# abeauvisage/uasl_motion_estimation

Measured on AMD Instinct MI355X. Metric: frames/sec + BA iter/sec, 2000 feats x 20-keyframe window, 1/2/4/8 MI355X, higher is better.
Workload: dtype u8+f32 (MI), f64 (BA); 1 GPU; config 3: 1280x720 stereo, 2000 feats, 20-keyframe window, 11x11 MI patches; frame=KLT + MI scale LM (LM, MAX_NB_ITER 10, tolerances off) + 10 BA LM iterations, parallelism=1 independent streams (one per GPU)

## Files before the change

### uasl_motion_estimation_amd/csrc/ba.hip

```cpp
#include <algorithm>
#include <cmath>
#include <cstdio>
#include <cstring>
#include <mutex>
#include <numeric>
#include <vector>
#include <hip/hip_ext.h>
#include "me_internal.hpp"
#include "ba_kernels.hpp"
#include "roster.hpp"
#include "solve_diag.hpp"
#include "me_device.hpp"

using me_dev::wave_sync;

using namespace ba;

namespace {

constexpr double kDblMin = 2.2250738585072014e-308;
constexpr double kDblEps = 2.220446049250313e-16;

template <int Ctrl>
__device__ __forceinline__ double dpp_f64(double x);
// ... 231 lines not shown
  __shared__ double lds[BLK / 64];
  const State* st = b.st;
  if (st->done || !st->need_lin) return;
  const int o = blockIdx.x * BLK + threadIdx.x;
  double cost = 0;
  if (o < g.no) {
    const int cur = st->cur;
    const int ci = b.cam_idx[o], pi = b.pt_idx[o];
    double r[4], Jc[24], Jp[12];
    obs_residual<OD>(g, b, o, b.cams[cur] + 6 * ci, b.pts[cur] + 3 * pi, r, Jc, Jp);
    const double s = r[0] * r[0] + r[1] * r[1] + r[2] * r[2] + r[3] * r[3];
    double rho0, sc;
    huber(s, &rho0, &sc);
    cost = 0.5 * rho0;
    for (int k = 0; k < 4; ++k) r[k] *= sc;
    for (int k = 0; k < 24; ++k) Jc[k] *= sc;
    for (int k = 0; k < 12; ++k) Jp[k] *= sc;
    const long slot = b.pos[o];
    double* X = b.obsx + slot * kObsxStride;
    X[0] = Jp[0] * Jp[0] + Jp[3] * Jp[3] + Jp[6] * Jp[6] + Jp[9] * Jp[9];
    X[1] = Jp[0] * Jp[1] + Jp[3] * Jp[4] + Jp[6] * Jp[7] + Jp[9] * Jp[10];
    X[2] = Jp[0] * Jp[2] + Jp[3] * Jp[5] + Jp[6] * Jp[8] + Jp[9] * Jp[11];
    X[3] = Jp[1] * Jp[1] + Jp[4] * Jp[4] + Jp[7] * Jp[7] + Jp[10] * Jp[10];
    X[4] = Jp[1] * Jp[2] + Jp[4] * Jp[5] + Jp[7] * Jp[8] + Jp[10] * Jp[11];
    X[5] = Jp[2] * Jp[2] + Jp[5] * Jp[5] + Jp[8] * Jp[8] + Jp[11] * Jp[11];
    for (int a = 0; a < 3; ++a) X[6 + a] = Jp[a] * r[0] + Jp[3 + a] * r[1] + Jp[6 + a] * r[2] + Jp[9 + a] * r[3];
    if (ci - g.nf >= 0) {
      double* W = b.Wo + 18 * slot;
      for (int a = 0; a < 6; ++a)
        for (int c = 0; c < 3; ++c)
          W[a * 3 + c] = Jc[a] * Jp[c] + Jc[6 + a] * Jp[3 + c] + Jc[12 + a] * Jp[6 + c] + Jc[18 + a] * Jp[9 + c];
    }
  }
  double v[1] = {cost};
  double out[1];
  block_sum<1>(v, out, lds);
  if (threadIdx.x == 0) b.part[R_COST * g.pstride + blockIdx.x] = out[0];
}

__device__ __forceinline__ bool last_arrival_wt(unsigned* cnt, unsigned expected) {
  __shared__ int slast;
  __syncthreads();
  if (threadIdx.x == 0) {
    asm volatile("s_waitcnt vmcnt(0)" ::: "memory");
    const unsigned k = __hip_atomic_fetch_add(cnt, 1u, ME_HO_RMW, __HIP_MEMORY_SCOPE_AGENT);
    slast = k == expected - 1;
    if (slast) __hip_atomic_store(cnt, 0u, __ATOMIC_RELAXED, __HIP_MEMORY_SCOPE_AGENT);
  }
  __syncthreads();
  return slast != 0;
}

__device__ void cam_reduce_body(const Geo& g, const Bufs& b, int sharded, const double* cpart, double* colnorm,
                                double* gc_raw, double* Uraw, int ci) {
  __shared__ double tot[27];
  __shared__ double csl[6];
  const State* st = b.st;
  const int u = threadIdx.x;
  if (u < 27) {
    double sum = 0.0;
    for (int k = 0; k < g.ck; ++k) sum += a_ld<true>(&cpart[27 * ((long)ci * g.ck + k) + u]);
    tot[u] = sum;
    if (u < 21) Uraw[21 * (long)ci + u] = sum;
    else gc_raw[6 * ci + u - 21] = sum;
  }
  __syncthreads();
  if (u < 6) {
    const int d = u * 6 - u * (u - 1) / 2;
    colnorm[6 * ci + u] = tot[d];
    if (!sharded) {
      double* cs = b.csc + 6 * ci;
      if (!st->scaled) cs[u] = g.jacobi ? 1.0 / (1.0 + sqrt(tot[d])) : 1.0;
      csl[u] = cs[u];
    }
  }
  if (sharded) return;
  __syncthreads();
  if (u < 21) {
    int a = 0, r = u;
    while (r >= 6 - a) {
      r -= 6 - a;
      ++a;
    }
    const int c = a + r;
    const double x = tot[u] * csl[a] * csl[c];
    double* U = b.U + 36 * (long)ci;
    U[a * 6 + c] = x;
    U[c * 6 + a] = x;
  } else if (u < 27) {
    b.gcs[6 * ci + u - 21] = tot[u] * csl[u - 21];
  }
}

#ifdef ME_CAM_TS
__device__ unsigned long long g_cam_ts[8];
#define CAM_T(i)                                                                           \
  do {                                                                                     \
    if (ci == 0 && k == 0 && threadIdx.x == 0) {                                           \
      const long long t_ = (long long)__builtin_amdgcn_s_memtime();                        \
      if ((i) > 0) atomicAdd(&g_cam_ts[(i)], (unsigned long long)(t_ - cam_prev_));        \
      else atomicAdd(&g_cam_ts[0], 1ull);                                                  \
      cam_prev_ = t_;                                                                      \
    }                                                                                      \
  } while (0)
#else
#define CAM_T(i) \
  do {           \
  } while (0)
#endif
template <int OD>
__device__ __forceinline__ void cam_assemble_body(const Geo& g, const Bufs& b, double* cpart, int sharded,
                                                  double* colnorm, double* gc_raw, double* Uraw, int ci, int k) {
  __shared__ double rows[kBlock / 16 * 27];
  const State* st = b.st;
  if (st->done || !st->need_lin) return;
#ifdef ME_CAM_TS
  long long cam_prev_ = 0;
#endif
  CAM_T(0);
  const int beg = b.c_off[ci], end = b.c_off[ci + 1];
  double v[27];
  for (int i = 0; i < 27; ++i) v[i] = 0;
  const int cur = st->cur;
  for (int q = beg + k * kBlock + threadIdx.x; q < end; q += g.ck * kBlock) {
    const int o = b.c_obs[q];
    const int cam = b.cam_idx[o], pi = b.pt_idx[o];
    double r[4], Jc[24], Jp[12];
    obs_residual<OD>(g, b, o, b.cams[cur] + 6 * cam, b.pts[cur] + 3 * pi, r, Jc, Jp);
    const double s2 = r[0] * r[0] + r[1] * r[1] + r[2] * r[2] + r[3] * r[3];
    double rho0, sc;
    huber(s2, &rho0, &sc);
    for (int kk = 0; kk < 4; ++kk) r[kk] *= sc;
    for (int kk = 0; kk < 24; ++kk) Jc[kk] *= sc;
    int u = 0;
    for (int a = 0; a < 6; ++a)
      for (int c = a; c < 6; ++c, ++u)
        v[u] += Jc[a] * Jc[c] + Jc[6 + a] * Jc[6 + c] + Jc[12 + a] * Jc[12 + c] + Jc[18 + a] * Jc[18 + c];
    for (int a = 0; a < 6; ++a) v[21 + a] += Jc[a] * r[0] + Jc[6 + a] * r[1] + Jc[12 + a] * r[2] + Jc[18 + a] * r[3];
  }
  CAM_T(1);
#pragma unroll
  for (int u = 0; u < 27; ++u) {
    double x = v[u];
    x += dpp_f64<kDppQuadSwap1>(x);
    x += dpp_f64<kDppQuadSwap2>(x);
    x += dpp_f64<kDppRowHalfMirror>(x);
    x += dpp_f64<kDppRowMirror>(x);
    v[u] = x;
  }
  if ((threadIdx.x & 15) == 0)
#pragma unroll
    for (int u = 0; u < 27; ++u) rows[(threadIdx.x >> 4) * 27 + u] = v[u];
  __syncthreads();
  CAM_T(2);
  if (threadIdx.x < 27) {
    double sum = 0.0;
#pragma unroll
    for (int r = 0; r < kBlock / 16; ++r) sum += rows[r * 27 + threadIdx.x];
    a_st<true>(&cpart[27 * ((long)ci * g.ck + k) + threadIdx.x], sum);
  }
  const bool last = last_arrival_wt(b.cnt + ci, g.ck);
  CAM_T(3);
  if (!last) return;
  cam_reduce_body(g, b, sharded, cpart, colnorm, gc_raw, Uraw, ci);
  CAM_T(4);
#ifdef ME_CAM_TS
  if (ci == 0 && k == 0 && threadIdx.x == 0) atomicAdd(&g_cam_ts[5], 1ull);
#endif
}

__global__ __launch_bounds__(kBlock) void cam_assemble_kernel(Geo g, Bufs b, double* cpart, int sharded,
                                                              double* colnorm, double* gc_raw, double* Uraw) {
  if (g.od == 4)
    cam_assemble_body<4>(g, b, cpart, sharded, colnorm, gc_raw, Uraw, blockIdx.x, blockIdx.y);
  else
    cam_assemble_body<2>(g, b, cpart, sharded, colnorm, gc_raw, Uraw, blockIdx.x, blockIdx.y);
}

struct CamArgs {
  double *cpart, *colnorm, *gc_raw, *Uraw;
  int on;
  int ncam;
};

__global__ void xch_flags_kernel(Geo g, Bufs b, double* colnorm) {
  colnorm[g.n6] = b.st->bad_input ? 1.0 : 0.0;
  colnorm[g.n6 + 1] = b.st->infeasible ? 1.0 : 0.0;
}

__global__ void cam_finish_kernel(Geo g, Bufs b, const double* colnorm, const double* gc_raw, const double* Uraw,
                                  int first) {
  State* st = b.st;
  if (first) {
    const bool bad = colnorm[g.n6] != 0.0, infeasible = colnorm[g.n6 + 1] != 0.0;
    __syncthreads();
    if (bad || infeasible) {
      if (blockIdx.x == 0 && threadIdx.x == 0) {
        st->bad_input = bad;
        st->infeasible = infeasible;
        st->done = 1;
        st->termination = 2;
      }
      return;
    }
  }
  if (st->done || !st->need_lin) return;
  const int ci = blockIdx.x * blockDim.x + threadIdx.x;
  if (ci >= g.m) return;
  double* cs = b.csc + 6 * ci;
  if (!st->scaled)
    for (int a = 0; a < 6; ++a) cs[a] = g.jacobi ? 1.0 / (1.0 + sqrt(colnorm[6 * ci + a])) : 1.0;
  const double* Ur = Uraw + 21 * (long)ci;
  double* U = b.U + 36 * (long)ci;
  int u = 0;
  for (int a = 0; a < 6; ++a)
    for (int c = a; c < 6; ++c, ++u) {
      const double x = Ur[u] * cs[a] * cs[c];
      U[a * 6 + c] = x;
      U[c * 6 + a] = x;
    }
  for (int a = 0; a < 6; ++a) b.gcs[6 * ci + a] = gc_raw[6 * ci + a] * cs[a];
}

__device__ __forceinline__ bool chol3(const double* A, double* L) {
  double d0 = A[0];
  if (!(d0 > 0)) return false;
  d0 = sqrt(d0);
  const double l10 = A[3] / d0, l20 = A[6] / d0;
  double d1 = A[4] - l10 * l10;
// ... 20 lines not shown
}

constexpr int kSchurPts = 16, kSchurPtsWide = 32, kSchurPtsSmall = 8;
#ifndef ME_SCHUR_NT
#define ME_SCHUR_NT 5
#endif
constexpr int kSchurNtMax = ME_SCHUR_NT;
constexpr size_t kSchurLdsCap = 150 * 1024;
__host__ __device__ inline size_t schur_lds_bytes(int P, int Rz) { return 8 * (size_t)3 * P * Rz + 4 * 3 * (size_t)P; }

template <int W>
__device__ __forceinline__ int group_min(int x) {
  if (W >= 2) x = min(x, dpp_i32<kDppQuadSwap1>(x));
  if (W >= 4) x = min(x, dpp_i32<kDppQuadSwap2>(x));
  if (W >= 8) x = min(x, dpp_i32<kDppRowHalfMirror>(x));
  if (W >= 16) x = min(x, dpp_i32<kDppRowMirror>(x));
  if (W >= 32) x = min(x, __shfl_xor(x, 16, W));
  if (W >= 64) x = min(x, __shfl_xor(x, 32, W));
  return x;
}
template <int W>
__device__ __forceinline__ int group_max(int x) {
  if (W >= 2) x = max(x, dpp_i32<kDppQuadSwap1>(x));
  if (W >= 4) x = max(x, dpp_i32<kDppQuadSwap2>(x));
  if (W >= 8) x = max(x, dpp_i32<kDppRowHalfMirror>(x));
  if (W >= 16) x = max(x, dpp_i32<kDppRowMirror>(x));
  if (W >= 32) x = max(x, __shfl_xor(x, 16, W));
  if (W >= 64) x = max(x, __shfl_xor(x, 32, W));
  return x;
}

#ifdef ME_SCHUR_STAMPS
#define SCHUR_T(i)                                                                     \
  do {                                                                                 \
    if (sblk == 0 && threadIdx.x == 0) {                                               \
      const long long tt_ = (long long)__builtin_amdgcn_s_memtime();                   \
      if ((i) > 0) st->stamps[5 + (i)] += tt_ - sch_prev_;                             \
      sch_prev_ = tt_;                                                                 \
    }                                                                                  \
  } while (0)
#else
#define SCHUR_T(i) \
  do {             \
  } while (0)
#endif
template <int NT, int BLK, int PTS>
__global__ __launch_bounds__(BLK) void pt_schur_kernel(Geo g, Bufs b, Opts o, CamArgs ca) {
  constexpr int SL = BLK / PTS, NW = BLK / 64;
  extern __shared__ double smem[];
  __shared__ double red[8];
  if (ca.on && (int)blockIdx.x < ca.ncam) {
    if (threadIdx.x >= kBlock) return;
    const int q = blockIdx.x;
    if (q >= g.m * g.ck) return;
    if (g.od == 4)
      cam_assemble_body<4>(g, b, ca.cpart, 0, ca.colnorm, ca.gc_raw, ca.Uraw, q / g.ck, q % g.ck);
    else
      cam_assemble_body<2>(g, b, ca.cpart, 0, ca.colnorm, ca.gc_raw, ca.Uraw, q / g.ck, q % g.ck);
    return;
  }
  const int sblk = (int)blockIdx.x - (ca.on ? ca.ncam : 0);
  State* st = b.st;
  if (st->done) return;
#ifdef ME_SCHUR_STAMPS
  long long sch_prev_ = 0;
  if (sblk == 0 && threadIdx.x == 0) st->stamps[12] += 1;
#endif
  SCHUR_T(0);
  const int need_lin = st->need_lin, scaled = st->scaled, cur = st->cur;
  const double* obsx = b.obsx;
  const double* Wo = b.Wo;
  const double radius = st->radius;
  const bool final_pass = st->iterations >= o.max_num_iterations;
  if (sblk == 0 && threadIdx.x == 0) st->final_pass = final_pass;
  const int P = g.spts, Rz = g.Rpad, rows = 3 * P, nks = rows / 4;
  const int sup = sblk / (8 * g.sgrp), r8 = sblk - sup * 8 * g.sgrp;
  const int run = 8 * sup + (r8 & 7), tgrp = r8 >> 3;
  if (run >= g.nruns) {
    if (need_lin && threadIdx.x == 0) b.part[R_GMAX_PT * g.pstride + sblk] = 0.0;
    return;
  }
  const int bA = g.sorted ? b.rband[2 * run] : 0, bB = g.sorted ? b.rband[2 * run + 1] : g.T - 1;
  const int nb = bB - bA + 1, ns = nb + (bB < g.T - 1 ? 1 : 0), ntile = ns * (ns + 1) / 2;
  if (tgrp * g.stpw >= ntile) {
    if (need_lin && threadIdx.x == 0) b.part[R_GMAX_PT * g.pstride + sblk] = 0.0;
    return;
  }
  const bool lead = tgrp == 0;
  double* Y = smem;
  int* band = reinterpret_cast<int*>(Y + (size_t)rows * Rz);
  const int tid = threadIdx.x, lane = tid & 63, wave = __builtin_amdgcn_readfirstlane(tid >> 6);
  const int gi = tid / SL, gl = tid & (SL - 1);
  int tI[NT], tJ[NT];
#pragma unroll
  for (int u = 0; u < NT; ++u) {
    int p = tgrp * g.stpw + wave + NW * u, ka = 0;
    if (p >= ntile) p = -1;
    int rem = p < 0 ? 0 : p;
    while (rem >= ns - ka) {
      rem -= ns - ka;
      ++ka;
    }
    const int kb = ka + rem;
    tI[u] = p < 0 ? -1 : (ka < nb ? bA + ka : g.T - 1);
    tJ[u] = p < 0 ? -1 : (kb < nb ? bA + kb : g.T - 1);
  }
  double4_t acc[NT];
#pragma unroll
  for (int u = 0; u < NT; ++u) acc[u] = double4_t{0.0, 0.0, 0.0, 0.0};
  double gm = 0;
  for (int sc = 0; sc < g.rsub; ++sc) {
// ... 1450 lines not shown
    double uy = 0.0;
#pragma unroll
    for (int k = 0; k < 6; ++k) uy += U[k] * y[k];
    cm += b.gcs[r] * yr + 0.5 * yr * uy;
  }
  double v3[3] = {s2, xn2, -cm}, out[3];
  block_sum<3>(v3, out, lds);
  if (tid == 0) {
    a_st<true>(&b.st->cam_step2, out[0]);
    a_st<true>(&b.st->cam_xn2, out[1]);
    a_st<true>(&b.st->cam_model, out[2]);
  }
}

template <int OD>
__global__ __launch_bounds__(kStepBlock) void pt_step_kernel(Geo g, Bufs b, Opts o, int do_decide) {
  __shared__ double lds[16];
  const State* st = b.st;
  if (blockIdx.x == 0 && threadIdx.x < 2) b.roster[threadIdx.x] = 0u;
  if (st->done) return;
#ifdef ME_STEP_TS
  long long step_prev_ = 0, fin_prev_ = 0;
#endif
  if ((int)blockIdx.x == g.nblk_step) {
    if (!st->fail) cam_step_body(g, b, st->cur, lds);
  } else {
  STEP_T(0);
  const int gl = threadIdx.x & (kStepG - 1);
  const int j = blockIdx.x * kStepPts + (threadIdx.x / kStepG);
  double mc = 0, cc = 0, s2 = 0, xn2 = 0;
  if (j < g.np && !st->fail) {
    const int cur = st->cur;
    const double* Wo = b.Wo;
    double psv[3], gpv[3], Lv[9], xv[3], Vv[9];
    for (int a = 0; a < 3; ++a) {
      psv[a] = b.psc[3 * (long)j + a];
      gpv[a] = b.gps[3 * (long)j + a];
      xv[a] = b.pts[cur][3 * (long)j + a];
    }
    for (int i = 0; i < 9; ++i) {
      Lv[i] = b.Lp[9 * (long)j + i];
      Vv[i] = b.V[9 * (long)j + i];
    }
    const int beg = b.p_off[j], end = b.p_off[j + 1];
    const int q0 = beg + gl;
    const bool has0 = q0 < end;
    int ci0 = -1, o0 = 0;
    double W0[18];
    if (has0) {
      ci0 = b.p_cam[q0];
      o0 = b.p_obs[q0];
      for (int i = 0; i < 18; ++i) W0[i] = Wo[18 * (long)q0 + i];
    }
    const double* cams_x = b.cams[cur];
    double ys0[6], f0[4];
    int cam0 = 0, right0 = 0;
    if (has0) {
      if (ci0 >= 0)
        for (int a = 0; a < 6; ++a) ys0[a] = b.csc[6 * ci0 + a] * b.yc[6 * ci0 + a];
      cam0 = ci0 + g.nf;
      for (int k = 0; k < OD; ++k) f0[k] = b.obs[(long)OD * o0 + k];
      if (OD == 2) right0 = b.cam_id[o0] != 0;
    }
    double cv0[6];
    if (has0)
      for (int a = 0; a < 6; ++a) {
        const double xa = cams_x[6 * cam0 + a];
        cv0[a] = ci0 >= 0 ? cam_cand(xa, ys0[a]) : xa;
      }
    STEP_T(1);
    double t[3] = {0.0, 0.0, 0.0};
    for (int q = q0; q < end; q += kStepG) {
      const bool first = q == q0;
      const int ci = first ? ci0 : b.p_cam[q];
      if (ci < 0) continue;
      double ys[6], W[18];
      if (first) {
        for (int a = 0; a < 6; ++a) ys[a] = ys0[a];
        for (int i = 0; i < 18; ++i) W[i] = W0[i];
      } else {
        for (int a = 0; a < 6; ++a) ys[a] = b.csc[6 * ci + a] * b.yc[6 * ci + a];
        for (int i = 0; i < 18; ++i) W[i] = Wo[18 * (long)q + i];
      }
      for (int c = 0; c < 3; ++c) {
        double s = 0;
        for (int a = 0; a < 6; ++a) s += W[a * 3 + c] * ys[a];
        t[c] += s;
      }
    }
    for (int c = 0; c < 3; ++c) t[c] = group_sum<kStepG>(t[c]);
    STEP_T(2);
    double rhs[3];
    for (int c = 0; c < 3; ++c) rhs[c] = -gpv[c] - t[c] * psv[c];
    double u[3], yp[3];
    fwd3(Lv, rhs, u);
    bwd3(Lv, u, yp);
    double d[3], xc[3];
    for (int a = 0; a < 3; ++a) {
      d[a] = yp[a] * psv[a];
      xc[a] = fmin(fmax(xv[a] + d[a], g.lo[a]), g.hi[a]);
    }
    if (gl == 0) {
      double gy = 0.0, yvy = 0.0, cross = 0.0;
      for (int a = 0; a < 3; ++a) {
        b.dp[3 * (long)j + a] = d[a];
        b.pts[1 - cur][3 * (long)j + a] = xc[a];
        const double dd = xc[a] - xv[a];
        s2 += dd * dd;
        xn2 += xv[a] * xv[a];
        gy += gpv[a] * yp[a];
        cross += d[a] * t[a];
        double vy = 0.0;
        for (int c = 0; c < 3; ++c) vy += Vv[3 * a + c] * yp[c];
        yvy += yp[a] * vy;
      }
      mc = -(gy + 0.5 * yvy + cross);
    }
    STEP_T(3);
    for (int q = q0; q < end; q += kStepG) {
      const bool first = q == q0;
      double cv[6], f[4];
      int right = 0;
      if (first) {
        for (int a = 0; a < 6; ++a) cv[a] = cv0[a];
        for (int k = 0; k < OD; ++k) f[k] = f0[k];
        right = right0;
      } else {
        const int o = b.p_obs[q];
        const int ci = b.p_cam[q], cam = ci + g.nf;
        for (int a = 0; a < 6; ++a) {
          const double xa = cams_x[6 * cam + a];
          cv[a] = ci >= 0 ? cam_cand(xa, b.csc[6 * ci + a] * b.yc[6 * ci + a]) : xa;
        }
        for (int k = 0; k < OD; ++k) f[k] = b.obs[(long)OD * o + k];
        if (OD == 2) right = b.cam_id[o] != 0;
      }
      double r[4];
      if (OD == 4)
        stereo_residual(g, cv, xc, f, r, nullptr, nullptr);
      else
        mono_residual(g, cv, xc, f, right, r, nullptr, nullptr);
      const double s = r[0] * r[0] + r[1] * r[1] + r[2] * r[2] + r[3] * r[3];
      double rho0, sc;
      huber(s, &rho0, &sc);
      cc += 0.5 * rho0;
    }
  }
  STEP_T(4);
  double v4[4] = {mc, cc, s2, xn2}, out[4];
  block_sum<4>(v4, out, lds);
  if (threadIdx.x == 0) {
    a_st<true>(&b.part[R_MODEL * g.pstride + blockIdx.x], out[0]);
    a_st<true>(&b.part[R_CAND * g.pstride + blockIdx.x], out[1]);
    a_st<true>(&b.part[R_STEP2 * g.pstride + blockIdx.x], out[2]);
    a_st<true>(&b.part[R_XN2 * g.pstride + blockIdx.x], out[3]);
  }
  STEP_T(5);
  }
  if (!last_arrival_wt(b.cnt + g.m, gridDim.x)) return;
#ifdef ME_STEP_TS
  if (threadIdx.x == 0) fin_prev_ = (long long)__builtin_amdgcn_s_memtime();
#endif
  step_finalize_body(g, b, o, do_decide);
  STEP_FIN_T(6);
#ifdef ME_STEP_TS
  if (threadIdx.x == 0) atomicAdd(&g_step_ts[7], 1ull);
#endif
}

__global__ void decide_kernel(Geo g, Bufs b, Opts o) {
  if (threadIdx.x != 0) return;
  if (b.st->done) return;
  decide(b, o);
}

template <int OD>
__global__ __launch_bounds__(kBlock) void cost_kernel(Geo g, Bufs b, int which, double* part) {
  __shared__ double lds[4];
  const int o = blockIdx.x * kBlock + threadIdx.x;
// ... 136 lines not shown
__global__ __launch_bounds__(kScanBlock) void plan_scan_kernel(Geo g, Bufs b, Opts o) {
  __shared__ int wsum[kScanBlock / 64];
  __shared__ int total;
  const PlanWork w = plan_work(g, b.work);
  const int t = threadIdx.x, lane = t & 63, wv = t >> 6;
  const int chunk = (g.np + kScanBlock - 1) / kScanBlock;
  const int beg = min(g.np, t * chunk), end = min(g.np, beg + chunk);
  int s = 0;
  for (int j = beg; j < end; ++j) s += w.cnt_p[j];
  int x = s;
  for (int off = 1; off < 64; off <<= 1) {
    const int y = __shfl_up(x, off, 64);
    if (lane >= off) x += y;
  }
  if (lane == 63) wsum[wv] = x;
  __syncthreads();
  if (t == 0) {
    int acc = 0;
    for (int k = 0; k < kScanBlock / 64; ++k) {
      const int v = wsum[k];
      wsum[k] = acc;
      acc += v;
    }
    total = acc;
  }
  __syncthreads();
  int run = wsum[wv] + x - s;
  for (int j = beg; j < end; ++j) {
    b.p_off[j] = run;
    run += w.cnt_p[j];
  }
  if (t == 0) b.p_off[g.np] = total;
  __shared__ int ctot[kMaxScanCams];
  const int bchunk = (g.nblk_obs + 63) / 64;
  for (int c = wv; c < g.m; c += kScanBlock / 64) {
    const int k0 = min(g.nblk_obs, lane * bchunk), k1 = min(g.nblk_obs, k0 + bchunk);
    int cs = 0;
    for (int k = k0; k < k1; ++k) cs += w.blk_cam[(long)k * g.nc + g.nf + c];
    int cx = cs;
    for (int off = 1; off < 64; off <<= 1) {
      const int y = __shfl_up(cx, off, 64);
      if (lane >= off) cx += y;
    }
    int r = cx - cs;
    for (int k = k0; k < k1; ++k) {
      int* e = &w.blk_cam[(long)k * g.nc + g.nf + c];
      const int v = *e;
      *e = r;
      r += v;
    }
    if (lane == 63) ctot[c] = cx;
  }
  __syncthreads();
  if (t == 0) {
    int acc = 0;
    for (int c = 0; c < g.m; ++c) {
      b.c_off[c] = acc;
      const int v = ctot[c];
      ctot[c] = acc;
      acc += v;
    }
    b.c_off[g.m] = acc;
  }
  __syncthreads();
  for (int c = wv; c < g.m; c += kScanBlock / 64) {
    const int k0 = min(g.nblk_obs, lane * bchunk), k1 = min(g.nblk_obs, k0 + bchunk);
    for (int k = k0; k < k1; ++k) w.blk_cam[(long)k * g.nc + g.nf + c] += ctot[c];
  }
  for (int i = t; i < g.n6; i += kScanBlock) b.csc[i] = 0.0;
  if (t == 0) {
    State* st = b.st;
    st->cur = 0;
    st->need_lin = 1;
    st->done = 0;
    st->termination = 1;
    st->iterations = st->successful = st->invalid_count = 0;
    st->fail = st->scaled = st->accepted = st->final_pass = st->spin_err = 0;
    st->bad_input = w.flags[F_BAD];
    st->infeasible = w.flags[F_INFEASIBLE];
    st->radius = o.initial_radius;
    st->decrease = 2.0;
    st->x_cost = st->cand_cost = st->model_change = st->initial_cost = 0.0;
    st->cam_step2 = st->cam_xn2 = st->cam_model = st->last_q = 0.0;
    for (int k = 0; k < 16; ++k) st->stamps[k] = 0;
    if (st->bad_input || st->infeasible) {
      st->done = 1;
      st->termination = 2;
    }
  }
}

__global__ __launch_bounds__(kBlock) void plan_scatter_kernel(Geo g, Bufs b) {
  __shared__ int scam[kBlock];
  const PlanWork w = plan_work(g, b.work);
  if (w.flags[F_BAD]) return;
  const int t = threadIdx.x, blk = blockIdx.x;
  const int o = blk * kBlock + t;
  const int ci = o < g.no ? b.cam_idx[o] : -1;
  scam[t] = ci;
  if (o < g.no) {
    const int pi = b.pt_idx[o];
    b.tmp_obs[b.p_off[pi] + atomicAdd(&w.fill_p[pi], 1)] = o;
  }
  __syncthreads();
  if (o < g.no) {
    int slot = -1;
    if (ci >= g.nf) {
      int rank = 0;
      for (int k = 0; k < t; ++k) rank += scam[k] == ci;
      slot = w.blk_cam[(long)blk * g.nc + ci] + rank;
      b.c_obs[slot] = o;
    }
    b.cpos[o] = slot;
  }
}

constexpr int kSortBlock = 256;
__global__ __launch_bounds__(kSortBlock) void plan_segsort_kernel(Geo g, Bufs b) {
  const PlanWork w = plan_work(g, b.work);
  if (w.flags[F_BAD]) return;
  const int lane = threadIdx.x & 63;
  const int j = blockIdx.x * (kSortBlock / 64) + (threadIdx.x >> 6);
  if (j >= g.np) return;
  const int beg = b.p_off[j], k = b.p_off[j + 1] - beg;
  auto key_of = [&](int o) { return ((unsigned long long)(unsigned)b.cam_idx[o] << 32) | (unsigned)o; };
  if (k <= 64) {
    const int o = lane < k ? b.tmp_obs[beg + lane] : 0;
    const unsigned long long key = lane < k ? key_of(o) : ~0ull;
    int rank = 0, same = 0;
    for (int l = 0; l < k; ++l) {
      const unsigned long long kl = __shfl(key, l, 64);
      rank += kl < key;
      same += (kl >> 32) == (key >> 32);
    }
    if (lane < k) {
      const int q = beg + rank;
      b.p_obs[q] = o;
// ... 208 lines not shown
inline int solve_form(int Ts) {
  if (8 * (solve_small_doubles(Ts) + solve_a_doubles(Ts)) <= kSolveLdsCap) return 0;
  return Ts >= kSolveMwMinTs ? 2 : 1;
}

extern "C" int me_debug_ba_geometry(int n_cams, int fixed_frames, int n_pts, int* out) {
  if (n_cams <= 0 || n_pts < 0 || !out) return ME_ERR_INVALID;
  Geo g;
  ba_geometry(g, n_cams, fixed_frames, n_pts);
  const int v[10] = {g.spts, g.nsub, g.rsub, g.rlen, g.nruns, g.stpw, g.sgrp, g.ksplit, g.sorted, solve_form(g.Ts)};
  std::memcpy(out, v, sizeof v);
  return ME_OK;
}

int ba_drain(me_ctx* c);

int plan_build(me_ctx* c, const me_ba_problem* p, const me_ba_options* opt, Plan& P, int slot_base,
               int async = -1, me_comm* comm = nullptr) {
  if (async < 0) ME_TRY(ba_drain(c));
  ME_CHECK(c, p->n_cams > 0 && p->n_pts >= 0 && p->n_obs >= 0, "BA: bad sizes");
  ME_CHECK(c, p->n_cams <= kMaxScanCams, "BA: at most %d cameras per window", kMaxScanCams);
  ME_CHECK(c, p->obs_dim == 0 || p->obs_dim == 2 || p->obs_dim == 4, "BA: obs_dim must be 2 or 4 (Observation<M>)");
  const bool mono = p->obs_dim == 2;
  ME_CHECK(c, p->feat_var > 0 && (mono || p->baseline != 0.0), "BA: wrong calibration parameters (BundleAdjuster.h:147)");
  ME_CHECK(c, !mono || p->cam_id || p->n_obs == 0, "BA: obs_dim 2 needs cam_id (Observation::camID)");
  const double baseline = mono && p->baseline == 0 ? 0.5 : p->baseline;
  ME_CHECK(c, p->mem == ME_HOST || p->mem == ME_DEVICE, "BA: bad memory kind");
  if (p->mem == ME_HOST) {
    for (int i = 0; i < p->n_obs; ++i) {
      ME_CHECK(c, p->cam_idx[i] >= 0 && p->cam_idx[i] < p->n_cams && p->pt_idx[i] >= 0 && p->pt_idx[i] < p->n_pts,
               "BA: observation %d indexes outside the window", i);
    }
  }
  P.c = c;
  int hook = c->dbg_solve_flags;
  if ((hook & kFlagFailEveryOther) && (c->dbg_solve_count++ & 1)) hook |= kFlagSolveFail;
  P.no_fused_asm = (hook & kFlagSeparateAsm) != 0;
  P.solve_flags = hook & (kFlagAsmTimeout | kFlagSolveFail | kFlagRosterNow);
  Geo& g = P.g;
  ba_geometry(g, p->n_cams, p->fixed_frames, p->n_pts);
  g.no = p->n_obs;
  g.od = mono ? 2 : 4;
  P.comm = comm;
  P.xmax_separate = comm && comm->world == 0;
  g.xslots = comm && comm->world > 0 ? comm->world : 1;
  g.xrank = comm && comm->world > 0 ? comm->rank : 0;
  ME_CHECK(c, g.nruns <= kMaxRuns, "BA: %d Schur runs exceed %d", g.nruns, kMaxRuns);
  g.nblkp = blocks(std::max(g.np, 1), kBlock);
  ME_CHECK(c, g.npairs <= 8 * 24, "BA: %d variable cameras exceed the Schur tile budget", g.m);
  g.nblk_obs = (int)std::max(1L, rup(std::max(g.no, 1), kBlock) / kBlock);
  g.nblk_lin = (int)std::max(1L, rup(std::max(g.no, 1), lin_block(g.no)) / lin_block(g.no));
  g.nblk_pts = (int)std::max(1L, rup(std::max(g.np, 1), kPtBlock) / kPtBlock);
  g.jacobi = opt->jacobi_scaling ? 1 : 0;
  g.ck = (int)std::min(64L, std::max(1L, rup(std::max(g.no, 1), (long)std::max(g.m, 1) * kBlock) /
                                             ((long)std::max(g.m, 1) * kBlock)));
  g.nblk_step = (int)std::max(1L, rup(std::max(g.np, 1), kStepPts) / kStepPts);
  g.pstride = std::max({g.nblk_obs, g.nblk_lin, g.nblk_pts, g.nblk_step, g.ksplit});
  std::memcpy(g.K0, p->K0, sizeof(g.K0));
  std::memcpy(g.K1, p->K1, sizeof(g.K1));
  g.baseline = baseline;
  g.sinv = 1.0 / std::sqrt(p->feat_var);
  const double Zmax = p->K0[0] * baseline / 0.1;
  const double Zmin = p->K0[0] * baseline / (2 * p->K0[2]);
  g.hi[0] = Zmax / p->K0[0] * p->K0[2];
  g.hi[1] = Zmax / p->K0[4] * p->K0[5];
  g.hi[2] = Zmax;
  g.lo[0] = -Zmax / p->K0[0] * p->K0[2];
  g.lo[1] = -Zmax / p->K0[4] * p->K0[5];
  g.lo[2] = Zmin;
  Opts& o = P.o;
  o.max_num_iterations = opt->max_num_iterations;
  o.function_tolerance = opt->function_tolerance;
  o.gradient_tolerance = opt->gradient_tolerance;
  o.parameter_tolerance = opt->parameter_tolerance;
  o.initial_radius = opt->initial_trust_region_radius;
  o.max_radius = opt->max_trust_region_radius;
  o.min_radius = opt->min_trust_region_radius;
  o.min_diag = opt->min_lm_diagonal;
  o.max_diag = opt->max_lm_diagonal;
  o.min_rel_decrease = opt->min_relative_decrease;
  o.max_invalid = opt->max_num_consecutive_invalid_steps;
  const bool dev = p->mem == ME_DEVICE;
  const long nb = g.pstride;
  Bufs& b = P.b;
  std::vector<std::pair<size_t, void**>> items;
  auto add = [&](size_t bytes, void* dst) { items.push_back({rup((long)std::max<size_t>(bytes, 8), 256), (void**)dst}); };
  add(8 * 6 * (size_t)g.nc, &b.cams[0]);
  add(8 * 3 * (size_t)g.np, &b.pts[0]);
  add(8 * g.od * (size_t)g.no, &b.obs);
  add(4 * (size_t)g.no, &b.cam_idx);
  add(4 * (size_t)g.no, &b.pt_idx);
  add(mono ? 4 * (size_t)g.no : 0, &b.cam_id);
  const size_t n_inputs = items.size();
  add(8 * 6 * (size_t)g.nc, &b.cams[1]);
  add(8 * 3 * (size_t)g.np, &b.pts[1]);
  add(4 * (size_t)(g.np + 1), &b.p_off);
  add(4 * (size_t)g.no, &b.p_obs);
  add(4 * (size_t)g.no, &b.pos);
  add(4 * (size_t)g.no, &b.p_cam);
  add(4 * (size_t)(g.m + 1), &b.c_off);
  add(4 * (size_t)g.no, &b.c_obs);
  add(4 * (size_t)g.no, &b.tmp_obs);
  add(4 * (size_t)g.no, &b.cpos);
  add(8 * kObsxStride * (size_t)g.no, &b.obsx);
  add((size_t)g.no, &b.dup);
  add(8 * solve_a_doubles(g.Ts), &b.Abuf);
  add(8 * 18 * (size_t)g.no, &b.Wo);
  add(8 * (size_t)g.n6, &b.csc);
  add(8 * 3 * (size_t)g.np, &b.psc);
  add(8 * 36 * (size_t)g.m, &b.U);
  add(8 * (size_t)g.n6, &b.gcs);
  add(8 * 9 * (size_t)g.np, &b.V);
  add(8 * 3 * (size_t)g.np, &b.gps);
  add(8 * 9 * (size_t)g.np, &b.Lp);
  add(8 * 3 * (size_t)g.np, &b.zp);
  add(8 * 256 * (size_t)g.nruns * g.npairs, &b.Spart);
  add(4 * (size_t)std::max(g.np, 1), &b.order);
  add(4 * (size_t)std::max(g.np, 1), &b.pkey);
  add(4 * (size_t)std::max(g.np, 1), &b.prank);
  add(4 * (size_t)g.T * g.T * g.nblkp, &b.phist);
  add(8 * (size_t)g.nruns, &b.rband);
  add(4 * (size_t)g.npairs * g.nruns, &b.tl);
  add(4 * (size_t)g.npairs, &b.tcnt);
  add(8 * (size_t)g.n6 * g.n6 + 8 * (size_t)(2 * g.n6 + 2), &b.S);
  add(8 * (size_t)g.n6, &b.yc);
  add(8 * 3 * (size_t)g.np, &b.dp);
  add(8 * R_COUNT * (size_t)nb, &b.part);
  add(8 * (R_COUNT + 2), &b.scal);
  add(sizeof(State), &b.st);
  add(8 * (size_t)(g.n6 + 2), &P.colnorm);
  add(8 * (size_t)g.n6, &P.gc_raw);
  add(8 * 21 * (size_t)std::max(g.m, 1), &P.Uraw);
  add(8 * 27 * (size_t)std::max(g.m, 1) * g.ck, &P.cpart);
  add(4 * (size_t)(g.m + 1 + 3 + 2), &b.cnt);
  add(4 * (size_t)blocks((long)g.npairs * 256, kSolveBlock / kSaGroups), &b.asm_claim);
  const size_t work_bytes = 4 * (2 * (size_t)g.np + (size_t)g.nblk_obs * g.nc + 4);
  add(work_bytes, &b.work);
  const size_t out_doubles = sizeof(State) / 8 + 6 * (size_t)g.nc + 3 * (size_t)g.np;
  add(8 * out_doubles, &b.out);
  b.xch = nullptr;
  if (comm) add(8 * (size_t)xo_total(g), &b.xch);
  size_t total = 0, input_span = 0;
  for (size_t k = 0; k < items.size(); ++k) {
    total += items[k].first;
    if (k < n_inputs) input_span += items[k].first;
  }
  void* arena;
  ME_TRY(me_scratch(c, SLOT_COUNT + slot_base, total, &arena));
  char* ptr = (char*)arena;
  for (auto& it : items) {
    *it.second = ptr;
    ptr += it.first;
  }
  b.ssync = b.cnt + g.m + 1;
  b.roster = b.cnt + g.m + 4;
  b.bvec = b.S + (size_t)g.n6 * g.n6;
  b.diagU = b.bvec + g.n6;
  void* hp;
  const size_t stage = rup((long)std::max(8 * out_doubles, dev ? (size_t)0 : input_span), 64);
  const size_t hbytes = stage + 2 * rup(sizeof(State), 64);
  if (async >= 0) {
    if (c->ba_pinned_size[async] < hbytes) {
      if (c->ba_pinned[async]) ME_HIP(c, hipHostFree(c->ba_pinned[async]));
      c->ba_pinned[async] = nullptr;
      c->ba_pinned_size[async] = 0;
      ME_HIP(c, hipHostMalloc(&c->ba_pinned[async], std::max(hbytes, (size_t)4096), hipHostMallocDefault));
      c->ba_pinned_size[async] = std::max(hbytes, (size_t)4096);
    }
    hp = c->ba_pinned[async];
  } else {
    ME_TRY(me_pinned(c, hbytes, &hp));
  }
  P.host = (double*)hp;
  if (P.reserve_only) return ME_OK;
  P.hstate[0] = (State*)((char*)hp + stage);
  P.hstate[1] = (State*)((char*)hp + stage + rup(sizeof(State), 64));
  P.dev = dev;
  hipStream_t s = c->stream;
  if (!dev) {
    char* h = (char*)hp;
    const void* src[6] = {p->cams, p->pts, p->obs, p->cam_idx, p->pt_idx, p->cam_id};
    const size_t len[6] = {8 * 6 * (size_t)g.nc, 8 * 3 * (size_t)g.np, 8 * g.od * (size_t)g.no, 4 * (size_t)g.no,
                           4 * (size_t)g.no, mono ? 4 * (size_t)g.no : 0};
    size_t off = 0;
    for (int k = 0; k < 6; ++k) {
      if (len[k]) std::memcpy(h + off, src[k], len[k]);
// ... 30 lines not shown
  if (!c->ba_lds_attr) {
    for (const void* k : {(const void*)cam_solve_kernel<0>, (const void*)cam_solve_kernel<1>, (const void*)cam_solve_kernel<2>})
      ME_HIP(c, hipFuncSetAttribute(k, hipFuncAttributeMaxDynamicSharedMemorySize, (int)kSolveLdsCap));
#define ME_SCHUR_K(N)                                                                                   \
  (const void*)pt_schur_kernel<N, 512, kSchurPts>, (const void*)pt_schur_kernel<N, 512, kSchurPtsWide>, \
      (const void*)pt_schur_kernel<N, 512, kSchurPtsSmall>
    for (const void* k : {ME_SCHUR_K(2), ME_SCHUR_K(3), ME_SCHUR_K(4), ME_SCHUR_K(5)})
#undef ME_SCHUR_K
      ME_HIP(c, hipFuncSetAttribute(k, hipFuncAttributeMaxDynamicSharedMemorySize, (int)kSchurLdsCap));
    c->ba_lds_attr = 1;
  }
  if (!P.use_lds) {
    int per_cu = 0;
    ME_HIP(c, hipOccupancyMaxActiveBlocksPerMultiprocessor(&per_cu, cam_solve_kernel<2>, kSolveBlock, P.solve_lds));
    P.solve_cap = std::max(0, per_cu) * (c->cu_active > 0 ? c->cu_active : c->num_cu);
    if (P.comm && g.Ts >= kSolveMwMinTs) {
      double* d = P.b.scal;
      const double v = -(double)P.solve_cap;
      ME_HIP(c, hipMemcpyAsync(d, &v, 8, hipMemcpyHostToDevice, c->stream));
      ME_TRY(me_comm_allreduce_impl(P.comm, d, 1, ME_COMM_MAX));
      double r = 0.0;
      ME_HIP(c, hipMemcpyAsync(&r, d, 8, hipMemcpyDeviceToHost, c->stream));
      ME_HIP(c, hipStreamSynchronize(c->stream));
      P.solve_cap = (int)-r;
    }
  }
  return ME_OK;
}



#define ME_XCH(ptr, n, op) ME_TRY(me_comm_allreduce_impl(P.comm, (ptr), (long)(n), (op)))

int enqueue_linearize(Plan& P) {
  me_ctx* c = P.c;
  const Geo& g = P.g;
  hipStream_t s = c->stream;
  const bool sh = P.comm != nullptr;
  {
    me_ktimer t(c, ME_KT_BA_LINEARIZE);
    const bool small = lin_block(g.no) == kLinSmall;
    if (g.od == 4 && small)
      hipLaunchKernelGGL((linearize_kernel<4, kLinSmall>), dim3(g.nblk_lin), dim3(kLinSmall), 0, s, g, P.b);
    else if (g.od == 4)
      hipLaunchKernelGGL((linearize_kernel<4, kBlock>), dim3(g.nblk_lin), dim3(kBlock), 0, s, g, P.b);
    else if (small)
      hipLaunchKernelGGL((linearize_kernel<2, kLinSmall>), dim3(g.nblk_lin), dim3(kLinSmall), 0, s, g, P.b);
    else
      hipLaunchKernelGGL((linearize_kernel<2, kBlock>), dim3(g.nblk_lin), dim3(kBlock), 0, s, g, P.b);
  }
  const bool first = P.n_enq == 0;
  const bool fused = !first && g.m > 0;
  ++P.n_enq;
  CamArgs ca{P.cpart, P.colnorm, P.gc_raw, P.Uraw, fused ? 1 : 0, fused ? (g.m * g.ck + 7) / 8 * 8 : 0};
  if (g.m > 0 && !fused)
    hipLaunchKernelGGL(cam_assemble_kernel, dim3(g.m, g.ck), dim3(kBlock), 0, s, g, P.b, P.cpart, sh ? 1 : 0,
                       P.colnorm, P.gc_raw, P.Uraw);
  if (sh && !fused) {
    if (first) {
      hipLaunchKernelGGL(xch_flags_kernel, dim3(1), dim3(1), 0, s, g, P.b, P.colnorm);
      ME_XCH(P.colnorm, g.n6 + 2, ME_COMM_SUM);
    }
    hipLaunchKernelGGL(cam_finish_kernel, dim3(blocks(std::max(g.m, 1), 64)), dim3(64), 0, s, g, P.b,
                       (const double*)P.colnorm, (const double*)P.gc_raw, (const double*)P.Uraw, first ? 1 : 0);
  }
  {
    me_ktimer t(c, ME_KT_BA_SCHUR, true);
    const int pw8 = g.stpw / 8;
    const dim3 grd(g.ksplit + ca.ncam);
#define ME_SCHUR(N)                                                                                          \
  do {                                                                                                       \
    if (g.spts == kSchurPtsWide)                                                                             \
      hipExtLaunchKernelGGL((pt_schur_kernel<N, 512, kSchurPtsWide>), grd, dim3(512), P.schur_lds, s, t.a, t.b, 0, g, \
                            P.b, P.o, ca);                                                                   \
    else if (g.spts == kSchurPtsSmall)                                                                       \
      hipExtLaunchKernelGGL((pt_schur_kernel<N, 512, kSchurPtsSmall>), grd, dim3(512), P.schur_lds, s, t.a, t.b, 0, g, \
                            P.b, P.o, ca);                                                                   \
    else                                                                                                     \
      hipExtLaunchKernelGGL((pt_schur_kernel<N, 512, kSchurPts>), grd, dim3(512), P.schur_lds, s, t.a, t.b, 0, g, P.b, \
                            P.o, ca);                                                                        \
  } while (0)
    static_assert(kSchurNtMax >= 3 && kSchurNtMax <= 5, "instantiated tile counts");
    if (pw8 <= 2) ME_SCHUR(2);
    else if (pw8 <= 3) ME_SCHUR(3);
    else if (pw8 <= 4) ME_SCHUR(4);
    else ME_SCHUR(5);
#undef ME_SCHUR
  }
  if (sh) {
    hipLaunchKernelGGL(s_assemble_kernel, dim3(blocks((long)g.npairs * 256, kSaElems) + 1), dim3(kBlock), 0, s, g,
                       P.b, P.o, (const double*)P.gc_raw, 0, (int)SA_PACK);
    if (P.xmax_separate) {
      ME_XCH(P.b.xch, xo_gmax(g), ME_COMM_SUM);
      ME_XCH(P.b.xch + xo_gmax(g), 1, ME_COMM_MAX);
    } else {
      ME_XCH(P.b.xch, xo_total(g), ME_COMM_SUM);
    }
  }
  return me_check_launch(c, "BA linearize");
}

int enqueue_assemble(Plan& P, bool img = false) {
  me_ctx* c = P.c;
  const Geo& g = P.g;
  const int mode = P.comm ? SA_UNPACK : SA_SUM;
  if (g.m > 0)
    hipLaunchKernelGGL(s_assemble_kernel, dim3(blocks((long)g.npairs * 256, kSaElems) + 1), dim3(kBlock), 0,
                       c->stream, g, P.b, P.o, (const double*)P.gc_raw, P.full_S ? 1 : 0, mode,
                       img && !P.full_S ? P.b.Abuf : nullptr);
// ... 647 lines not shown
__global__ void window_indices_kernel(const int32_t* __restrict__ frame, const int32_t* __restrict__ ids, int n_obs,
                                      int f0, const int32_t* __restrict__ win_ids, int n_pts,
                                      int32_t* __restrict__ cam_idx, int32_t* __restrict__ pt_idx) {
  const int i = blockIdx.x * blockDim.x + threadIdx.x;
  if (i >= n_obs) return;
  const int32_t id = ids[i];
  int lo = 0, hi = n_pts;
  while (lo < hi) {
    const int mid = (lo + hi) >> 1;
    if (win_ids[mid] < id) lo = mid + 1;
    else hi = mid;
  }
  cam_idx[i] = frame[i] - f0;
  pt_idx[i] = (lo < n_pts && win_ids[lo] == id) ? lo : -1;
}

extern "C" int me_ba_window_indices(me_ctx* c, const int32_t* frame, const int32_t* ids, int n_obs, int first_frame,
                                    const int32_t* win_ids, int n_pts, int32_t* cam_idx, int32_t* pt_idx) {
  if (!c) return ME_ERR_INVALID;
  ME_CHECK(c, n_obs >= 0 && n_pts >= 0, "me_ba_window_indices: bad sizes");
  if (n_obs == 0) return ME_OK;
  ME_HIP(c, hipSetDevice(c->device));
  hipLaunchKernelGGL(window_indices_kernel, dim3(blocks(n_obs, kBlock)), dim3(kBlock), 0, c->stream, frame, ids, n_obs,
                     first_frame, win_ids, n_pts, cam_idx, pt_idx);
  return me_check_launch(c, "window_indices_kernel");
}

extern "C" int me_debug_solve_flags(me_ctx* c, int flags) {
  if (!c) return ME_ERR_INVALID;
  ME_CHECK(c, (flags & ~kHookMask) == 0, "me_debug_solve_flags: 0x%x holds bits that are no test hook (accepted: 0x%x)",
           (unsigned)flags, (unsigned)kHookMask);
  c->dbg_solve_flags = flags;
  c->dbg_solve_count = 0;
  return ME_OK;
}

extern "C" int me_debug_read(me_ctx* c, long long* out, int n) {
  if (!c || n < 0 || n > 16) return ME_ERR_INVALID;
  std::memcpy(out, c->dbg, 8 * (size_t)n);
  return ME_OK;
}

#ifdef ME_CAM_TS
extern "C" int me_cam_ts(long long* out, int reset) {
  unsigned long long h[8];
  if (hipMemcpyFromSymbol(h, HIP_SYMBOL(g_cam_ts), sizeof h) != hipSuccess) return -1;
  for (int i = 0; i < 8; ++i) out[i] = (long long)h[i];
  if (reset) {
    const unsigned long long z[8] = {0, 0, 0, 0, 0, 0, 0, 0};
    if (hipMemcpyToSymbol(HIP_SYMBOL(g_cam_ts), z, sizeof z) != hipSuccess) return -1;
  }
  return 0;
}
#endif

#ifdef ME_STEP_TS
extern "C" int me_step_ts(long long* out, int reset) {
  unsigned long long h[12];
  if (hipMemcpyFromSymbol(h, HIP_SYMBOL(g_step_ts), sizeof h) != hipSuccess) return -1;
  for (int i = 0; i < 12; ++i) out[i] = (long long)h[i];
  if (reset) {
    const unsigned long long z[12] = {0, 0, 0, 0, 0, 0, 0, 0, 0, 0, 0, 0};
    if (hipMemcpyToSymbol(HIP_SYMBOL(g_step_ts), z, sizeof z) != hipSuccess) return -1;
  }
  return 0;
}
#endif
```

### uasl_motion_estimation_amd/csrc/ba_kernels.hpp

```cpp
#pragma once
#include <hip/hip_runtime.h>
#include <stdint.h>

namespace ba {

typedef double double4_t __attribute__((ext_vector_type(4)));

constexpr int kBlock = 256;
constexpr int kObsxStride = 9;

struct Opts {
  int max_num_iterations;
  double function_tolerance, gradient_tolerance, parameter_tolerance;
  double initial_radius, max_radius, min_radius, min_diag, max_diag, min_rel_decrease;
  int max_invalid;
};

struct State {
  int cur;
  int need_lin;
  int done;
  int termination;
  int iterations, successful, invalid_count;
  int fail;
  int scaled;
  int accepted;
  int bad_input;
  int infeasible;
  int final_pass;
  int spin_err;
  int pad[2];
  double radius, decrease;
  double x_cost, cand_cost, model_change, initial_cost;
  double cam_step2, cam_xn2, cam_model;
  double last_q;
  long long stamps[16];
};

enum { R_COST = 0, R_GMAX_PT, R_MODEL, R_CAND, R_STEP2, R_XN2, R_COUNT };

struct Geo {
  int nc, np, no, nf, m, n6, Rpad, T, Ts, spts, nsub, ksplit, npairs, nblk_obs, nblk_lin, nblk_pts, nblk_step, pstride, jacobi,
      ck;
  int nruns, rlen, rsub, sgrp, stpw, nblkp;
  int sorted;
  int od;
  int xslots, xrank;
  double K0[9], K1[9];
  double baseline, sinv;
  double lo[3], hi[3];
};

struct Bufs {
  double* cams[2];
  double* pts[2];
  const double* obs;
  const int* cam_idx;
  const int* pt_idx;
  const int* cam_id;
  int* p_off;
  int* p_obs;
  int* pos;
  int* p_cam;
  int* c_off;
  int* c_obs;
  int* tmp_obs;
  int* cpos;
  double* obsx;
  uint8_t* dup;
  double* Abuf;
  double* Wo;
  double* csc;
  double* psc;
  double* U;
  double* gcs;
  double* V;
  double* gps;
  double* Lp;
  double* zp;
  double* Spart;
  int* order;
  int* rband;
  int* tl;
  int* tcnt;
  int* pkey;
  int* prank;
  int* phist;
  double* S;
  double* bvec;
  double* diagU;
  double* yc;
  double* dp;
  double* part;
  double* scal;
  State* st;
  int* work;
  unsigned* cnt;
  unsigned* ssync;
  unsigned* roster;
  unsigned* asm_claim;
  double* out;
  double* xch;
};

__host__ __device__ inline long xo_diag(const Geo& g) { return (long)g.npairs * 256; }
__host__ __device__ inline long xo_gc(const Geo& g) { return xo_diag(g) + g.n6; }
__host__ __device__ inline long xo_cost(const Geo& g) { return xo_gc(g) + g.n6; }
__host__ __device__ inline long xo_fail(const Geo& g) { return xo_cost(g) + 1; }
__host__ __device__ inline long xo_gmax(const Geo& g) { return xo_fail(g) + 1; }
__host__ __device__ inline long xo_total(const Geo& g) { return xo_gmax(g) + g.xslots; }

}
```

Before: 1344 frames/s.

## Replace fixed per-camera block split with variable work-unit table for camera assembly

Camera Hessian assembly used a uniform grid of m x ck blocks, each striding over a camera's observations, so load was uneven when cameras have different observation counts. A unit table built in the scan kernel now assigns each block exactly one 256-observation chunk of one camera, with per-camera unit counts driving the last-arrival reduction. The step kernel also prefetches the second observation's camera data ahead of the loop. This adds a small table write and extra indirection per block, and launches more blocks when cameras have many observations.

```diff
diff --git a/uasl_motion_estimation_amd/csrc/ba.hip b/uasl_motion_estimation_amd/csrc/ba.hip
--- a/uasl_motion_estimation_amd/csrc/ba.hip
+++ b/uasl_motion_estimation_amd/csrc/ba.hip
@@ -307,14 +307,14 @@
 }
 
 __device__ void cam_reduce_body(const Geo& g, const Bufs& b, int sharded, const double* cpart, double* colnorm,
-                                double* gc_raw, double* Uraw, int ci) {
+                                double* gc_raw, double* Uraw, int ci, int first, int count) {
   __shared__ double tot[27];
   __shared__ double csl[6];
   const State* st = b.st;
   const int u = threadIdx.x;
   if (u < 27) {
     double sum = 0.0;
-    for (int k = 0; k < g.ck; ++k) sum += a_ld<true>(&cpart[27 * ((long)ci * g.ck + k) + u]);
+    for (int k = 0; k < count; ++k) sum += a_ld<true>(&cpart[27 * ((long)first + k) + u]);
     tot[u] = sum;
     if (u < 21) Uraw[21 * (long)ci + u] = sum;
     else gc_raw[6 * ci + u - 21] = sum;
@@ -349,9 +349,10 @@
 
 #ifdef ME_CAM_TS
 __device__ unsigned long long g_cam_ts[8];
+__device__ int g_cam_ts_unit;
 #define CAM_T(i)                                                                           \
   do {                                                                                     \
-    if (ci == 0 && k == 0 && threadIdx.x == 0) {                                           \
+    if (un == g_cam_ts_unit && threadIdx.x == 0) {                                         \
       const long long t_ = (long long)__builtin_amdgcn_s_memtime();                        \
       if ((i) > 0) atomicAdd(&g_cam_ts[(i)], (unsigned long long)(t_ - cam_prev_));        \
       else atomicAdd(&g_cam_ts[0], 1ull);                                                  \
@@ -365,19 +366,23 @@
 #endif
 template <int OD>
 __device__ __forceinline__ void cam_assemble_body(const Geo& g, const Bufs& b, double* cpart, int sharded,
-                                                  double* colnorm, double* gc_raw, double* Uraw, int ci, int k) {
+                                                  double* colnorm, double* gc_raw, double* Uraw, int un) {
   __shared__ double rows[kBlock / 16 * 27];
   const State* st = b.st;
+  const int4 ue = *(const int4*)(b.cunit + (long)kCuStride * un);
+  const int ufirst = b.cunit[(long)kCuStride * un + CU_FIRST];
   if (st->done || !st->need_lin) return;
+  const int ci = ue.x;
+  if (ci < 0) return;
 #ifdef ME_CAM_TS
   long long cam_prev_ = 0;
 #endif
   CAM_T(0);
-  const int beg = b.c_off[ci], end = b.c_off[ci + 1];
   double v[27];
   for (int i = 0; i < 27; ++i) v[i] = 0;
   const int cur = st->cur;
-  for (int q = beg + k * kBlock + threadIdx.x; q < end; q += g.ck * kBlock) {
+  const int q = ue.y + threadIdx.x;
+  if (q < ue.z) {
     const int o = b.c_obs[q];
     const int cam = b.cam_idx[o], pi = b.pt_idx[o];
     double r[4], Jc[24], Jp[12];
@@ -412,24 +417,24 @@
     double sum = 0.0;
 #pragma unroll
     for (int r = 0; r < kBlock / 16; ++r) sum += rows[r * 27 + threadIdx.x];
-    a_st<true>(&cpart[27 * ((long)ci * g.ck + k) + threadIdx.x], sum);
-  }
-  const bool last = last_arrival_wt(b.cnt + ci, g.ck);
+    a_st<true>(&cpart[27 * (long)un + threadIdx.x], sum);
+  }
+  const bool last = last_arrival_wt(b.cnt + ci, (unsigned)ue.w);
   CAM_T(3);
   if (!last) return;
-  cam_reduce_body(g, b, sharded, cpart, colnorm, gc_raw, Uraw, ci);
+  cam_reduce_body(g, b, sharded, cpart, colnorm, gc_raw, Uraw, ci, ufirst, ue.w);
   CAM_T(4);
 #ifdef ME_CAM_TS
-  if (ci == 0 && k == 0 && threadIdx.x == 0) atomicAdd(&g_cam_ts[5], 1ull);
+  if (un == g_cam_ts_unit && threadIdx.x == 0) atomicAdd(&g_cam_ts[5], 1ull);
 #endif
 }
 
 __global__ __launch_bounds__(kBlock) void cam_assemble_kernel(Geo g, Bufs b, double* cpart, int sharded,
                                                               double* colnorm, double* gc_raw, double* Uraw) {
   if (g.od == 4)
-    cam_assemble_body<4>(g, b, cpart, sharded, colnorm, gc_raw, Uraw, blockIdx.x, blockIdx.y);
+    cam_assemble_body<4>(g, b, cpart, sharded, colnorm, gc_raw, Uraw, blockIdx.x);
   else
-    cam_assemble_body<2>(g, b, cpart, sharded, colnorm, gc_raw, Uraw, blockIdx.x, blockIdx.y);
+    cam_assemble_body<2>(g, b, cpart, sharded, colnorm, gc_raw, Uraw, blockIdx.x);
 }
 
 struct CamArgs {
@@ -556,11 +561,14 @@
   if (ca.on && (int)blockIdx.x < ca.ncam) {
     if (threadIdx.x >= kBlock) return;
     const int q = blockIdx.x;
-    if (q >= g.m * g.ck) return;
+    if (q >= g.ncu) return;
+#ifdef ME_EXP_NOCAM
+    return;
+#endif
     if (g.od == 4)
-      cam_assemble_body<4>(g, b, ca.cpart, 0, ca.colnorm, ca.gc_raw, ca.Uraw, q / g.ck, q % g.ck);
+      cam_assemble_body<4>(g, b, ca.cpart, 0, ca.colnorm, ca.gc_raw, ca.Uraw, q);
     else
-      cam_assemble_body<2>(g, b, ca.cpart, 0, ca.colnorm, ca.gc_raw, ca.Uraw, q / g.ck, q % g.ck);
+      cam_assemble_body<2>(g, b, ca.cpart, 0, ca.colnorm, ca.gc_raw, ca.Uraw, q);
     return;
   }
   const int sblk = (int)blockIdx.x - (ca.on ? ca.ncam : 0);
@@ -2117,6 +2125,13 @@
       o0 = b.p_obs[q0];
       for (int i = 0; i < 18; ++i) W0[i] = Wo[18 * (long)q0 + i];
     }
+    const int q1 = q0 + kStepG;
+    const bool has1 = q1 < end;
+    int ci1 = -1, o1 = 0;
+    if (has1) {
+      ci1 = b.p_cam[q1];
+      o1 = b.p_obs[q1];
+    }
     const double* cams_x = b.cams[cur];
     double ys0[6], f0[4];
     int cam0 = 0, right0 = 0;
@@ -2127,22 +2142,39 @@
       for (int k = 0; k < OD; ++k) f0[k] = b.obs[(long)OD * o0 + k];
       if (OD == 2) right0 = b.cam_id[o0] != 0;
     }
-    double cv0[6];
+    double ys1[6], f1[4];
+    int cam1 = 0, right1 = 0;
+    if (has1) {
+      if (ci1 >= 0)
+        for (int a = 0; a < 6; ++a) ys1[a] = b.csc[6 * ci1 + a] * b.yc[6 * ci1 + a];
+      cam1 = ci1 + g.nf;
+      for (int k = 0; k < OD; ++k) f1[k] = b.obs[(long)OD * o1 + k];
+      if (OD == 2) right1 = b.cam_id[o1] != 0;
+    }
+    double cv0[6], cv1[6];
     if (has0)
       for (int a = 0; a < 6; ++a) {
         const double xa = cams_x[6 * cam0 + a];
         cv0[a] = ci0 >= 0 ? cam_cand(xa, ys0[a]) : xa;
       }
+    if (has1)
+      for (int a = 0; a < 6; ++a) {
+        const double xa = cams_x[6 * cam1 + a];
+        cv1[a] = ci1 >= 0 ? cam_cand(xa, ys1[a]) : xa;
+      }
     STEP_T(1);
     double t[3] = {0.0, 0.0, 0.0};
     for (int q = q0; q < end; q += kStepG) {
-      const bool first = q == q0;
-      const int ci = first ? ci0 : b.p_cam[q];
+      const bool first = q == q0, second = q == q1;
+      const int ci = first ? ci0 : second ? ci1 : b.p_cam[q];
       if (ci < 0) continue;
       double ys[6], W[18];
       if (first) {
         for (int a = 0; a < 6; ++a) ys[a] = ys0[a];
         for (int i = 0; i < 18; ++i) W[i] = W0[i];
+      } else if (second) {
+        for (int a = 0; a < 6; ++a) ys[a] = ys1[a];
+        for (int i = 0; i < 18; ++i) W[i] = Wo[18 * (long)q + i];
       } else {
         for (int a = 0; a < 6; ++a) ys[a] = b.csc[6 * ci + a] * b.yc[6 * ci + a];
         for (int i = 0; i < 18; ++i) W[i] = Wo[18 * (long)q + i];
@@ -2183,13 +2215,17 @@
     }
     STEP_T(3);
     for (int q = q0; q < end; q += kStepG) {
-      const bool first = q == q0;
+      const bool first = q == q0, second = q == q1;
       double cv[6], f[4];
       int right = 0;
       if (first) {
         for (int a = 0; a < 6; ++a) cv[a] = cv0[a];
         for (int k = 0; k < OD; ++k) f[k] = f0[k];
         right = right0;
+      } else if (second) {
+        for (int a = 0; a < 6; ++a) cv[a] = cv1[a];
+        for (int k = 0; k < OD; ++k) f[k] = f1[k];
+        right = right1;
       } else {
         const int o = b.p_obs[q];
         const int ci = b.p_cam[q], cam = ci + g.nf;
@@ -2432,21 +2468,38 @@
     if (lane == 63) ctot[c] = cx;
   }
   __syncthreads();
+  __shared__ int ufst[kMaxScanCams + 1];
+  __shared__ int ctotal;
   if (t == 0) {
-    int acc = 0;
+    int acc = 0, units = 0;
     for (int c = 0; c < g.m; ++c) {
       b.c_off[c] = acc;
       const int v = ctot[c];
       ctot[c] = acc;
       acc += v;
+      ufst[c] = units;
+      units += max(1, (v + kBlock - 1) / kBlock);
     }
     b.c_off[g.m] = acc;
+    ctotal = acc;
+    ufst[g.m] = units;
   }
   __syncthreads();
   for (int c = wv; c < g.m; c += kScanBlock / 64) {
     const int k0 = min(g.nblk_obs, lane * bchunk), k1 = min(g.nblk_obs, k0 + bchunk);
     for (int k = k0; k < k1; ++k) w.blk_cam[(long)k * g.nc + g.nf + c] += ctot[c];
-  }
+    const int cbeg = ctot[c], cend = c + 1 < g.m ? ctot[c + 1] : ctotal;
+    const int first = ufst[c], count = ufst[c + 1] - first;
+    for (int k = lane; k < count; k += 64) {
+      int* e = b.cunit + (long)kCuStride * (first + k);
+      e[CU_CAM] = c;
+      e[CU_BEG] = cbeg + k * kBlock;
+      e[CU_END] = min(cend, cbeg + (k + 1) * kBlock);
+      e[CU_COUNT] = count;
+      e[CU_FIRST] = first;
+    }
+  }
+  for (int u = ufst[g.m] + t; u < (g.ncu + 7) / 8 * 8; u += kScanBlock) b.cunit[(long)kCuStride * u + CU_CAM] = -1;
   for (int i = t; i < g.n6; i += kScanBlock) b.csc[i] = 0.0;
   if (t == 0) {
     State* st = b.st;
@@ -2463,6 +2516,7 @@
     st->x_cost = st->cand_cost = st->model_change = st->initial_cost = 0.0;
     st->cam_step2 = st->cam_xn2 = st->cam_model = st->last_q = 0.0;
     for (int k = 0; k < 16; ++k) st->stamps[k] = 0;
+    st->stamps[14] = ufst[g.m];
     if (st->bad_input || st->infeasible) {
       st->done = 1;
       st->termination = 2;
@@ -2777,8 +2831,7 @@
   g.nblk_lin = (int)std::max(1L, rup(std::max(g.no, 1), lin_block(g.no)) / lin_block(g.no));
   g.nblk_pts = (int)std::max(1L, rup(std::max(g.np, 1), kPtBlock) / kPtBlock);
   g.jacobi = opt->jacobi_scaling ? 1 : 0;
-  g.ck = (int)std::min(64L, std::max(1L, rup(std::max(g.no, 1), (long)std::max(g.m, 1) * kBlock) /
-                                             ((long)std::max(g.m, 1) * kBlock)));
+  g.ncu = (int)(rup(std::max(g.no, 1), kBlock) / kBlock) + g.m;
   g.nblk_step = (int)std::max(1L, rup(std::max(g.np, 1), kStepPts) / kStepPts);
   g.pstride = std::max({g.nblk_obs, g.nblk_lin, g.nblk_pts, g.nblk_step, g.ksplit});
   std::memcpy(g.K0, p->K0, sizeof(g.K0));
@@ -2856,7 +2909,8 @@
   add(8 * (size_t)(g.n6 + 2), &P.colnorm);
   add(8 * (size_t)g.n6, &P.gc_raw);
   add(8 * 21 * (size_t)std::max(g.m, 1), &P.Uraw);
-  add(8 * 27 * (size_t)std::max(g.m, 1) * g.ck, &P.cpart);
+  add(8 * 27 * (size_t)g.ncu, &P.cpart);
+  add(4 * (size_t)kCuStride * (size_t)rup(g.ncu, 8), &b.cunit);
   add(4 * (size_t)(g.m + 1 + 3 + 2), &b.cnt);
   add(4 * (size_t)blocks((long)g.npairs * 256, kSolveBlock / kSaGroups), &b.asm_claim);
   const size_t work_bytes = 4 * (2 * (size_t)g.np + (size_t)g.nblk_obs * g.nc + 4);
@@ -2993,9 +3047,9 @@
   const bool first = P.n_enq == 0;
   const bool fused = !first && g.m > 0;
   ++P.n_enq;
-  CamArgs ca{P.cpart, P.colnorm, P.gc_raw, P.Uraw, fused ? 1 : 0, fused ? (g.m * g.ck + 7) / 8 * 8 : 0};
+  CamArgs ca{P.cpart, P.colnorm, P.gc_raw, P.Uraw, fused ? 1 : 0, fused ? (g.ncu + 7) / 8 * 8 : 0};
   if (g.m > 0 && !fused)
-    hipLaunchKernelGGL(cam_assemble_kernel, dim3(g.m, g.ck), dim3(kBlock), 0, s, g, P.b, P.cpart, sh ? 1 : 0,
+    hipLaunchKernelGGL(cam_assemble_kernel, dim3(g.ncu), dim3(kBlock), 0, s, g, P.b, P.cpart, sh ? 1 : 0,
                        P.colnorm, P.gc_raw, P.Uraw);
   if (sh && !fused) {
     if (first) {
@@ -3749,6 +3803,10 @@
   }
   return 0;
 }
+extern "C" int me_cam_ts_unit(int unit) {
+  if (unit < 0) return -1;
+  return hipMemcpyToSymbol(HIP_SYMBOL(g_cam_ts_unit), &unit, sizeof unit) == hipSuccess ? 0 : -1;
+}
 #endif
 
 #ifdef ME_STEP_TS
diff --git a/uasl_motion_estimation_amd/csrc/ba_kernels.hpp b/uasl_motion_estimation_amd/csrc/ba_kernels.hpp
--- a/uasl_motion_estimation_amd/csrc/ba_kernels.hpp
+++ b/uasl_motion_estimation_amd/csrc/ba_kernels.hpp
@@ -41,7 +41,7 @@
 
 struct Geo {
   int nc, np, no, nf, m, n6, Rpad, T, Ts, spts, nsub, ksplit, npairs, nblk_obs, nblk_lin, nblk_pts, nblk_step, pstride, jacobi,
-      ck;
+      ncu;
   int nruns, rlen, rsub, sgrp, stpw, nblkp;
   int sorted;
   int od;
@@ -66,6 +66,7 @@
   int* c_obs;
   int* tmp_obs;
   int* cpos;
+  int* cunit;
   double* obsx;
   uint8_t* dup;
   double* Abuf;
@@ -103,6 +104,9 @@
   double* xch;
 };
 
+constexpr int kCuStride = 8;
+enum { CU_CAM = 0, CU_BEG, CU_END, CU_COUNT, CU_FIRST };
+
 __host__ __device__ inline long xo_diag(const Geo& g) { return (long)g.npairs * 256; }
 __host__ __device__ inline long xo_gc(const Geo& g) { return xo_diag(g) + g.n6; }
 __host__ __device__ inline long xo_cost(const Geo& g) { return xo_gc(g) + g.n6; }
```

Result: faster. 1361 frames/s (median of 6 runs) (+1.2%).
